# ttanida/rgrg

Measured on AMD Instinct MI355X. Metric: images/sec full 29-region report gen, 512x512 CXR, greedy max_len=128, higher is better.
Workload: dtype bf16; 1 GPU; full_model.generate() batch=32/GPU, 29 regions, greedy max_len=128, bf16 autocast: 16-bit detector, 16-bit decode GEMMs + K/V cache, hipGraph-captured decode step (BASELINE configs[2]); global_batch=32, parallelism=single GPU, weights=seeded random init (rgrg_amd.synth, profile bench), hipGraph_decode=True

## Files before the change

### include/rgrg_hip.h

```cpp
#ifndef RGRG_HIP_H_
#define RGRG_HIP_H_

#include <stdint.h>

#ifdef __cplusplus
extern "C" {
#endif

#define RGRG_OK 0
#define RGRG_EINVAL (-1)
#define RGRG_EHIP (-2)
#define RGRG_ESTATE (-3)

#define RGRG_ACT_NONE 0
#define RGRG_ACT_RELU 1
#define RGRG_ACT_GELU_NEW 2

const char* rgrg_last_error(void);
int rgrg_abi_version(void);
int rgrg_device_arch(int dev, char* buf, int buflen);

int rgrg_linear_f32(const float* A, const float* W, const float* scale, const float* shift, const float* R,
                    float* Y, int M, int N, int K, int ldy, int act, int splitk, float* ws, void* stream);
int rgrg_conv2d_nhwc_f32(const float* X, const float* W, const float* scale, const float* shift, const float* R,
// ... 143 lines not shown
int rgrg_linear_bf16w_f32(const float* A, const uint16_t* Wb, const float* shift, const float* R, float* Y, int M,
                          int N, int K, int ldy, int act, int fp16, void* stream);
int rgrg_linear_bf16_f32(const uint16_t* A16, const uint16_t* Wb, const float* shift, const float* R, float* Y,
                         uint16_t* Y16, int M, int N, int K, int ldy, int act, int fp16, void* stream);
int rgrg_debug_linear_bf16_tile(const uint16_t* A16, const uint16_t* Wb, const float* shift, const float* R, float* Y,
                                int M, int N, int K, int ldy, int act, int tile, int lda, int ldw, int fp16, void* stream);
int rgrg_debug_conv2d_nhwc_bf16_tile(const uint16_t* X16, const uint16_t* Wb, const float* shift, const uint16_t* R16, float* Y,
                                     uint16_t* Y16, int B, int H, int Wd, int Cin, int Cout, int KH, int KW, int stride,
                                     int pad, int act, int fp16, int tile, void* stream);
int rgrg_debug_bf16_tile_choice(int M, int N, int K);
int rgrg_debug_linear_bf16_train(const uint16_t* A16, const uint16_t* Wb, const float* shift, const float* R, float* Y,
                                 uint16_t* Y16, uint16_t* Ypre16, const uint16_t* G16, int M, int N, int K, int ldy, int act,
                                 int tile, int fp16, void* stream);
int rgrg_debug_linear_bf16_argmax(const uint16_t* A16, const uint16_t* Wb, const float* shift, int M, int N, int K,
                                  float* cand_val, int* cand_idx, int fp16, void* stream);
int rgrg_debug_ln_fold16(const float* w, const float* gain, const float* beta, const float* bias, uint16_t* wb, float* colsum,
                         float* shift, int N, int K, int fp16, void* stream);
int rgrg_debug_linear_bf16_ln(const uint16_t* A16, const uint16_t* Wb, const float* shift, const float* R, float* Y,
                              uint16_t* Yb16, float* stats_out, const float* ln_stats, const float* ln_colsum, int M, int N,
                              int K, int ldy, int act, int fp16, void* stream);
int rgrg_debug_linear_bf16_ln_kv(const uint16_t* A16, const uint16_t* Wb, const float* shift, float* Y, const float* ln_stats,
                                 const float* ln_colsum, uint16_t* kcache, uint16_t* vcache, const int* step_dev, int M, int H,
                                 int T_slots, int K, int ldy, int fp16, void* stream);
int rgrg_debug_linear_bf16_ln_kp(const uint16_t* A16, const uint16_t* Wb, const float* shift, const float* R, float* Y,
                                 uint16_t* Y16, uint16_t* Yb16, float* stats_out, const float* ln_stats, const float* ln_colsum,
                                 int M, int N, int K, int ldy, int act, int fp16, int kp, void* stream);
int rgrg_debug_wide_epilogue_launches(void);
int rgrg_debug_cons_epilogue_launches(void);
int rgrg_debug_attn_decode(const float* qkv, int ld_qkv, void* kcache, void* vcache, const int* step_dev, float* out,
                           uint16_t* out16, int S, int H, int T_slots, const int* src, const float* kmask, int kv16, int fp16,
// ... 98 lines not shown
```

### rgrg_amd/_hip.py

```python
from __future__ import annotations

import ctypes as C
import os
from typing import Optional

from . import build as _build

c_float_p = C.c_void_p
_i, _f, _p = C.c_int, C.c_float, C.c_void_p

ACT_NONE, ACT_RELU, ACT_GELU_NEW = 0, 1, 2
ABI_VERSION = 28


class RgrgHipError(RuntimeError):
    pass


class DecoderLayerWeights(C.Structure):
    _fields_ = [(n, _p) for n in ("ln1_g", "ln1_b", "ln2_g", "ln2_b", "c_attn_w", "c_attn_b", "attn_proj_w",
                                  "attn_proj_b", "c_fc_w", "c_fc_b", "mlp_proj_w", "mlp_proj_b")]


class DirectArgs(C.Structure):
# ... 63 lines not shown
    "rgrg_colsum_f32": (_i, [_p, _p, _i, _i, _p]),
    "rgrg_relu_backward_f32": (_i, [_p, _p, C.c_int64, _p]),
    "rgrg_bce_with_logits_masked_backward_f32": (_i, [_p, _p, _p, C.c_float, _i, C.c_float, _p, _i, _p]),
    "rgrg_adamw_step_f32": (_i, [_p, _p, _p, _p, C.c_int64, C.c_float, C.c_float, C.c_float, C.c_float, C.c_float, _i, C.c_float, _p]),
    "rgrg_adamw_multi_step_f32": (_i, [_p, _i, C.c_float, C.c_float, C.c_float, C.c_float, C.c_float, _i, C.c_float, _p]),
    "rgrg_f32_to_bf16": (_i, [_p, _p, C.c_int64, _i, _p]),
    "rgrg_bf16_to_f32": (_i, [_p, _p, C.c_int64, _i, _p]),
    "rgrg_conv2d_nhwc_bf16": (_i, [_p, _p, _p, _p, _p, _p, _i, _i, _i, _i, _i, _i, _i, _i, _i, _i, _i, _p]),
    "rgrg_linear_bf16w_f32": (_i, [_p, _p, _p, _p, _p, _i, _i, _i, _i, _i, _i, _p]),
    "rgrg_linear_bf16_f32": (_i, [_p, _p, _p, _p, _p, _p, _i, _i, _i, _i, _i, _i, _p]),
    "rgrg_debug_linear_bf16_tile": (_i, [_p, _p, _p, _p, _p, _i, _i, _i, _i, _i, _i, _i, _i, _i, _p]),
    "rgrg_debug_conv2d_nhwc_bf16_tile": (_i, [_p, _p, _p, _p, _p, _p, _i, _i, _i, _i, _i, _i, _i, _i, _i, _i, _i, _i, _p]),
    "rgrg_debug_bf16_tile_choice": (_i, [_i, _i, _i]),
    "rgrg_debug_linear_bf16_train": (_i, [_p, _p, _p, _p, _p, _p, _p, _p, _i, _i, _i, _i, _i, _i, _i, _p]),
    "rgrg_debug_linear_bf16_argmax": (_i, [_p, _p, _p, _i, _i, _i, _p, _p, _i, _p]),
    "rgrg_debug_ln_fold16": (_i, [_p, _p, _p, _p, _p, _p, _p, _i, _i, _i, _p]),
    "rgrg_debug_direct_pack": (_i, [_p, _p, _p, _p, _i, _i, _i, _p, _p, _p, _p, _p, _p]),
    "rgrg_debug_direct_linear": (_i, [C.POINTER(DirectArgs), _i, _i, _i, _i, C.POINTER(_i), _p]),
    "rgrg_debug_skinny_linear": (_i, [_p, _p, _p, _p, _p, _i, _i, _i, _i, _i, _p]),
    "rgrg_debug_linear_bf16_ln": (_i, [_p, _p, _p, _p, _p, _p, _p, _p, _p, _i, _i, _i, _i, _i, _i, _p]),
    "rgrg_debug_linear_bf16_ln_kp": (_i, [_p, _p, _p, _p, _p, _p, _p, _p, _p, _p, _i, _i, _i, _i, _i, _i, _i, _p]),
    "rgrg_debug_wide_epilogue_launches": (_i, []),
    "rgrg_debug_cons_epilogue_launches": (_i, []),
    "rgrg_debug_attn_decode": (_i, [_p, _i, _p, _p, _p, _p, _p, _i, _i, _i, _p, _p, _i, _i, _i, _i, _i, _p]),
    "rgrg_debug_linear_bf16_ln_kv": (_i, [_p, _p, _p, _p, _p, _p, _p, _p, _p, _i, _i, _i, _i, _i, _i, _p]),
    "rgrg_debug_attn_decode_qonly": (_i, [_p, _i, _p, _p, _p, _p, _p, _i, _i, _i, _i, _i, _p]),
    "rgrg_debug_attn_decode_first": (_i, [_p, _i, _p, _p, _p, _p, _p, _i, _i, _i, _p, _i, _i, _i, _p]),
    "rgrg_debug_attn_decode_rowstep": (_i, [_p, _i, _p, _p, _p, _p, _p, _i, _i, _i, _i, _i, _i, _i, _p]),
    "rgrg_debug_attn_decode_beam_first": (_i, [_p, _i, _p, _p, _p, _p, _p, _i, _i, _i, _p, _p, _i, _i, _i, _i, _p]),
    "rgrg_debug_attn_decode_kv8": (_i, [_p, _i, _p, _p, _p, _p, _p, _i, _i, _i, _p, _p, _i, _i, _p]),
# ... 82 lines not shown
```

### rgrg_amd/csrc/decoder.hip

```cpp
#include <math.h>
#include <stdlib.h>

#include <algorithm>
#include <type_traits>
#include <cmath>
#include <vector>

#include "decoder_internal.h"

namespace rgrg {

int skinny_max_rows() {
    static int v = -1;
    if (v < 0) { const char* e = getenv("RGRG_SKINNY_MAX_ROWS"); v = e ? atoi(e) : SKINNY_MAX_ROWS;
        if (v > SKINNY_MAX_ROWS) v = SKINNY_MAX_ROWS; if (v < 32) v = 32; }
    return v;
}

__global__ __launch_bounds__(256) void pack_weights_kernel(const float* __restrict__ W, float* __restrict__ P, int N,
                                                           int K, int NT) {
    const size_t total = (size_t)NT * (K / 8) * 64;
    for (size_t o = (size_t)blockIdx.x * blockDim.x + threadIdx.x; o < total; o += (size_t)gridDim.x * blockDim.x) {
        const int l = (int)(o & 63);
        const size_t t = o >> 6;
// ... 1184 lines not shown
    return kv_is_bf16(d, S) && d->xn16 && d->ln_fold && d->ln_stat && d->layers[0].c_attn.wb_ln && d->D == 1024;
}
static bool step_qkv_cache(const rgrg_decoder* d, const StepSpec& s) {
    const int S = s.rows;
    const KvFormat f = kv_format(d, S);
    const bool plain = !s.tok && !s.src;
    return d->qkv_cache && plain && step_ln_fold(d, S) && (f == KV_BF16 || f == KV_F16) && d->kp_gemms != 1 && d->kp_gemms != 3 && !s.key_mask;
}
static GemmLnFold cons_kv_cache(const rgrg_decoder* d, const GemmLnFold& cons, int l, int r0) {
    GemmLnFold f = cons;
    u16* kcr = reinterpret_cast<u16*>(d->kv) + (size_t)l * d->kv_layer_stride + (size_t)r0 * d->H * d->T * 64;
    f.kv_k = kcr; f.kv_v = kcr + d->kv_kv_stride; f.kv_step = d->step; f.kv_H = d->H; f.kv_T = d->T;
    return f;
}

static int enqueue_head(rgrg_decoder* d, int S, bool count, bool logits, unsigned short* xn16, bool roll = false) {
    hipStream_t st = d->stream;
    int rc;
    if (!logits && xn16 && lm_head_cand_path(d, S)) {
        GemmLnFold ce{};
        ce.cand_val = d->cand_val; ce.cand_idx = d->cand_idx;
        if ((rc = linear(d, d->lm_head, d->xn, nullptr, nullptr, S, d->ld_logits, RGRG_ACT_NONE, count, xn16, nullptr, &ce))) return rc;
        if ((rc = trace_mark(d, 0, 1002))) return rc;
        if (roll) return enqueue_roll_end(d, S, (d->lm_head.N + 255) / 256);
        hipLaunchKernelGGL(argmax_update_kernel, dim3(S), dim3(256), 0, st, d->cand_val, d->cand_idx, (d->lm_head.N + 255) / 256, d->ids,
                           d->max_len, d->finished, d->step, d->done_len, d->sync, S);
        RGRG_LAUNCH_CHECK();
        return trace_mark(d, 0, 1003);
    }
    if ((rc = linear(d, d->lm_head, d->xn, nullptr, d->logits, S, d->ld_logits, RGRG_ACT_NONE, count, xn16))) return rc;
    if (logits) return RGRG_OK;
    const int cand_nt = (d->V + 31) / 32;
    hipLaunchKernelGGL(logits_candidates_kernel, dim3(4, S), dim3(256), 0, st, d->logits, d->ld_logits, d->V,
                       cand_nt, d->cand_val, d->cand_idx);
    RGRG_LAUNCH_CHECK();
    if (roll) return enqueue_roll_end(d, S, cand_nt);
    hipLaunchKernelGGL(argmax_update_kernel, dim3(S), dim3(256), 0, st, d->cand_val, d->cand_idx, cand_nt, d->ids,
                       d->max_len, d->finished, d->step, d->done_len, d->sync, S);
    RGRG_LAUNCH_CHECK();
    return RGRG_OK;
// ... 66 lines not shown
            if (!fold) {
                if ((rc2 = launch_ln_rows(x, w.ln2_g, w.ln2_b, xn, D, xn16r, d->f16(), rows, rs))) return rc2;
            }
            if ((rc2 = linear(d, w.c_fc, xn, nullptr, d->ff + 4 * o, rows, 4 * D, RGRG_ACT_GELU_NEW, count, xn16r, ff16r, cfr))) return rc2;
            if ((rc2 = trace_mark(d, r0, l * 8 + 3))) return rc2;
            if ((rc2 = linear(d, w.mlp_proj, d->ff + 4 * o, x, x, rows, D, RGRG_ACT_NONE, count, ff16r, nullptr, pfr))) return rc2;
            if ((rc2 = trace_mark(d, r0, l * 8 + 4))) return rc2;
            if (!fold || l + 1 == d->n_layer) {
                if ((rc2 = launch_ln_rows(x, ng, nb, xn, D, xn16r, d->f16(), rows, rs))) return rc2;
                if ((rc2 = trace_mark(d, r0, 1001))) return rc2;
            }
        }
        return RGRG_OK;
    };
    if ((rc = run_row_ranges(d, S, step_chains(d, S, s.end == STEP_ARGMAX && !s.tok && !s.src, fold), run_rows))) return rc;
    return enqueue_head(d, S, count, s.end != STEP_ARGMAX && s.end != STEP_ROLL, xn16, s.end == STEP_ROLL);
}
int enqueue_step(rgrg_decoder* d, const StepSpec& s, bool count) {
    const int rc = s.rows <= decode_row_limit(d) ? enqueue_step_fused(d, s, count) : enqueue_step_tiled(d, s, count);
    if (rc) return rc;
    if (s.end == STEP_SAMPLE) return enqueue_sampler(d, s.rows);
    return s.end == STEP_ROLL_SAMPLE ? enqueue_roll_sample_end(d, s.rows) : RGRG_OK;
}

StepSpec padded_step_spec(rgrg_decoder* d, StepSpec s, const int* pad) {
    s.row_pos = d->row_pos;
    if (kv_format(d, s.rows) != KV_F32) s.kv_first = pad;
    else s.key_mask = d->key_mask;
    return s;
}

// ... 820 lines not shown
                }
                const GemmLnFold cons_kv = qc ? cons_kv_cache(d, cons_r, l, r0) : cons_r;
                if ((rc2 = linear(d, w.c_attn, d->xn + o, nullptr, d->qkv + 3 * o, rows, 3 * D, RGRG_ACT_NONE, c, xn16r, nullptr, qc ? &cons_kv : cfr))) break;
                if ((rc2 = linear(d, w.attn_proj, d->att + o, d->x + o, d->h1 + o, rows, D, RGRG_ACT_NONE, c, att16r, nullptr, pfr))) break;
                if ((rc2 = linear(d, w.c_fc, d->xn + o, nullptr, d->ff + 4 * o, rows, 4 * D, RGRG_ACT_GELU_NEW, c, xn16r, ff16r, cfr))) break;
                if ((rc2 = linear(d, w.mlp_proj, d->ff + 4 * o, d->x + o, d->h1 + o, rows, D, RGRG_ACT_NONE, c, ff16r, nullptr, pfr))) break;
            }
            return rc2;
        });
        if (!rc && fused) {
            DirectArgs h{};
            h.Xf = d->x; h.part = d->part; h.Y = d->logits; h.ldy = d->ld_logits; h.act = RGRG_ACT_NONE;
            rc = direct_linear(d, d->lm_head, h, DX_COMBINE4, S, c, true);
        } else if (!rc) {
            if (xn16 && lm_head_cand_path(d, S)) {
                GemmLnFold ce{};
                ce.cand_val = d->cand_val; ce.cand_idx = d->cand_idx;
                rc = linear(d, d->lm_head, d->xn, nullptr, nullptr, S, d->ld_logits, RGRG_ACT_NONE, c, xn16, nullptr, &ce);
            } else {
                rc = linear(d, d->lm_head, d->xn, nullptr, d->logits, S, d->ld_logits, RGRG_ACT_NONE, c, xn16);
            }
        }
    }
    if (!rc) {
        RGRG_HIP(hipEventRecord(e1, d->stream));
        RGRG_HIP(hipEventSynchronize(e1));
        RGRG_HIP(hipEventElapsedTime(&tg, e0, e1));
        hipLaunchKernelGGL(set_int_kernel, dim3(1), dim3(64), 0, d->stream, d->step, nkeys - 2);
        for (int it = -1; it < iters && !rc; ++it) {
            if (it == 0) RGRG_HIP(hipEventRecord(e0, d->stream));
            rc = run_row_ranges(d, S, fused ? 1 : step_chains(d, S, true, fold), [&](int r0, int rows) -> int {
                int rc2 = RGRG_OK;
                for (int l = 0; l < d->n_layer && !rc2; ++l)
// ... 53 lines not shown
```

### rgrg_amd/csrc/gemm_bf16.hip

```cpp
#include "gemm_bf16_device.h"

#include <atomic>

namespace rgrg {

struct GemmBf16Params {
    const float* A;
    const u16* A16;
    const u16* Wb;
    const float* shift;
    const float* R;
    float* Y;
    u16* Y16;
    int M, N, K, ldy, act;
    int lda = 0, ldw = 0;
    int cH = 0, cW = 0, cCin = 0, cKH = 0, cKW = 0, cStride = 1, cPad = 0, cOH = 0, cOW = 0;
    const u16* R16 = nullptr;
    int f16 = 0;
    u16* Yb16 = nullptr;
    float* stats_out = nullptr;
    const float* ln_stats = nullptr;
    const float* ln_colsum = nullptr;
    u16 *kv_k = nullptr, *kv_v = nullptr;
    const int* kv_step = nullptr;
    int kv_H = 0, kv_T = 0;
    u16* Ypre16 = nullptr;
    const u16* G16 = nullptr;
    int gm = 0;
    int ksplit = 0;
    float* sk_ws = nullptr;
    unsigned* sk_cnt = nullptr;
    float* cand_val = nullptr;
    int* cand_idx = nullptr;
    int dbg = 0;
};

constexpr int BK16 = 64;
constexpr int LDB = (BK16 * 2 + 16) / 2;

template <int BM, int BN, int THREADS, bool A16, bool F16>
__global__ __launch_bounds__(THREADS) void gemm_bf16w_kernel(const GemmBf16Params p, const int mtiles, const int ntiles) {
    constexpr int WAVES = THREADS / 64, WN = WAVES / 2;
    constexpr int TM = BM / 2, TN = BN / WN;
    constexpr int MI = TM / 32, NI = TN / 32;
    constexpr int AL = BM * 8 / THREADS, BL = BN * 8 / THREADS;
    constexpr int RSTEP = THREADS / 8;
    constexpr int NS = 4;
    extern __shared__ __attribute__((aligned(16))) u16 smem16[];
// ... 180 lines not shown
    __builtin_amdgcn_sched_group_barrier(0x008, MI * NI, 0);
    __builtin_amdgcn_sched_group_barrier(0x100, MI + NI, 0);
    __builtin_amdgcn_sched_group_barrier(0x008, MI * NI, 0);
    __builtin_amdgcn_sched_group_barrier(0x008, MI * NI, 0);
}

template <int BM, int BN, int NST, bool CONV, bool F16, int LNF, int CACT = -1>
__global__ __launch_bounds__(256) void gemm_bf16_glds_kernel(const GemmBf16Params p, const int mtiles, const int ntiles) {
    constexpr int BK = 64;
    constexpr int MI = BM / 64, NI = BN / 64;
    constexpr int LA = BM / 32, LB = BN / 32;
    constexpr int LPW = LA + LB;
    constexpr int STAGE = (BM + BN) * 128;
    static_assert((NST - 2) * LPW < 64, "counted vmcnt out of range");
    static_assert(NST >= 2 && NST <= 4, "tail is written for up to 3 trailing tiles");
    constexpr bool CONS = LNF >= 2, KVC = LNF == 3;
    static_assert(CACT == -1 || (CONS && BM == 64 && BN == 64), "compile-time activation: consumers on the 64 x 64 tile");
    constexpr int ETAG = (CACT + 1) * 256;
    extern __shared__ __attribute__((aligned(16))) unsigned char glds_smem[];
    const int tid = threadIdx.x, lane = tid & 63;
    const int wave = __builtin_amdgcn_readfirstlane(tid >> 6);
    const int wm = wave >> 1, wn = wave & 1;
    const int ks = (!CONV && p.ksplit > 1) ? p.ksplit : 1;
    const int t = xcd_band_tile(blockIdx.x, mtiles * ntiles * ks);
    const int slice = t % ks, tile = t / ks;
    const int2 tmn = grouped_tile(tile, p.gm, mtiles, ntiles);
    const int tm = tmn.x, tn = tmn.y;
    const int m0 = tm * BM, n0 = tn * BN;
    const int nk = p.K / BK / ks;
    const int lda = p.lda ? p.lda : p.K, ldw = p.ldw ? p.ldw : p.K;
    const u16* abase = CONV ? p.A16 - 128 : p.A16 + (size_t)m0 * lda + (size_t)slice * nk * BK;
    const u16* wbase = p.Wb + (size_t)n0 * ldw + (size_t)slice * nk * BK;
    const int lrow = lane >> 3, lch = lane & 7;
    int va[LA], vb[LB];
    int cy0[LA], cx0[LA], cpix[LA], cswz[LA];
#pragma unroll
    for (int j = 0; j < LA; ++j) {
        const int row = (j * 4 + wave) * 8 + lrow;
// ... 37 lines not shown
    for (int ks = 0; ks < 4; ++ks) foff[ks] = frag_offset(frow, fh, ks);

    f32x16 acc[MI][NI];
    zero_acc(acc);

    const int ccol = lane & 31, crow4 = 4 * (lane >> 5);
    float sh_pre[MI][NI], cs_pre[MI][NI];
#pragma unroll
    for (int mi = 0; mi < MI; ++mi)
#pragma unroll
        for (int ni = 0; ni < NI; ++ni) {
            const int colc = min(n0 + wn * (BN / 2) + ni * 32 + ccol, p.N - 1);
            sh_pre[mi][ni] = p.shift ? p.shift[colc] : 0.f;
            cs_pre[mi][ni] = CONS ? p.ln_colsum[colc] : 0.f;
        }
    constexpr bool PRE_R = MI * NI == 1 && !CONS;
    float rv_pre[16];
#pragma unroll
    for (int r = 0; r < 16; ++r) rv_pre[r] = 0.f;
    if constexpr (PRE_R) {
        if (p.R) {
            const int colc = min(n0 + wn * (BN / 2) + ccol, p.N - 1);
            const int rbase = m0 + wm * (BM / 2) + crow4;
#pragma unroll
            for (int r = 0; r < 16; ++r) rv_pre[r] = c_load_f32(p.R, rbase, r, colc, p.M, p.ldy);
        }
    }

    constexpr int TPR = 256 / BM, PER = 16 / TPR;
    f32x4 lsq[PER / 2];
    int kv_slot = 0;
// ... 23 lines not shown
        nxt = nxt + 1 == NST ? 0 : nxt + 1;
    }
#define RGRG_GLDS_TAIL(R)                                   \
    if constexpr (NST - 1 >= (R)) {                         \
        wait_vmcnt<((R) - 1) * LPW>();                      \
        __builtin_amdgcn_s_barrier();                       \
        __builtin_amdgcn_sched_barrier(0);                  \
        RGRG_GLDS_COMPUTE(cur);                             \
        cur = cur + 1 == NST ? 0 : cur + 1;                 \
    }
    RGRG_GLDS_TAIL(3) RGRG_GLDS_TAIL(2) RGRG_GLDS_TAIL(1)
#undef RGRG_GLDS_TAIL
#undef RGRG_GLDS_ISSUE
#undef RGRG_GLDS_COMPUTE

    if constexpr (!CONV) {
        if (ks > 1) {
            const __amdgpu_buffer_rsrc_t rs = bf16_rsrc(p.sk_ws + (size_t)tile * ks * (BM * BN));
            const int soff = slice * (BM * BN * 4);
#pragma unroll
            for (int mi = 0; mi < MI; ++mi)
#pragma unroll
                for (int ni = 0; ni < NI; ++ni)
#pragma unroll
                    for (int q = 0; q < 4; ++q)
                        __builtin_amdgcn_raw_buffer_store_b128(
                            __builtin_bit_cast(u32x4, f32x4{acc[mi][ni][4 * q], acc[mi][ni][4 * q + 1], acc[mi][ni][4 * q + 2], acc[mi][ni][4 * q + 3]}),
                            rs, (((mi * NI + ni) * 4 + q) * 256 + tid) * 16, soff, 16);
            asm volatile("s_waitcnt vmcnt(0)" ::: "memory");
            __syncthreads();
            unsigned* flag = reinterpret_cast<unsigned*>(glds_smem + NST * STAGE + BM * 8);
// ... 6 lines not shown
#pragma unroll
                for (int ni = 0; ni < NI; ++ni)
#pragma unroll
                    for (int q = 0; q < 4; ++q) {
                        f32x4 tot = {0.f, 0.f, 0.f, 0.f};
                        for (int sl = 0; sl < ks; ++sl) {
                            f32x4 v = __builtin_bit_cast(f32x4, __builtin_amdgcn_raw_buffer_load_b128(rs, (((mi * NI + ni) * 4 + q) * 256 + tid) * 16,
                                                                                                         sl * (BM * BN * 4), 16));
                            if (sl == slice) v = f32x4{acc[mi][ni][4 * q], acc[mi][ni][4 * q + 1], acc[mi][ni][4 * q + 2], acc[mi][ni][4 * q + 3]};
                            tot += v;
                        }
#pragma unroll
                        for (int e = 0; e < 4; ++e) acc[mi][ni][4 * q + e] = tot[e];
                    }
        }
    }

    float2* row_stat = reinterpret_cast<float2*>(glds_smem + NST * STAGE);
    if constexpr (CONS) {
        const float2 ls = ln_slot_sums<TPR, PER>(lsq);
        const float mean = ln_mean(ls.x), var = ln_var(ls.y, mean);
        if (tid % TPR == 0) row_stat[tid / TPR] = make_float2(mean, 1.0f / sqrtf(var + LN_EPS16));
        __syncthreads();
    }

    float blk1[MI], blk2[MI];
#pragma unroll
    for (int mi = 0; mi < MI; ++mi) { blk1[mi] = 0.f; blk2[mi] = 0.f; }
#pragma unroll
    for (int mi = 0; mi < MI; ++mi)
// ... 306 lines not shown
                cv[(g * 4 + wq) * 128 + lrow_t] = bv[0];
                ci[(g * 4 + wq) * 128 + lrow_t] = bi[0];
            }
        }
        __syncthreads();
        if (tid < 256) {
            const int gg = tid >> 7, lr = tid & 127, row = m0 + tid;
            float best = cv[(gg * 4) * 128 + lr];
            int idx = ci[(gg * 4) * 128 + lr];
#pragma unroll
            for (int q = 1; q < 4; ++q) {
                const float v = cv[(gg * 4 + q) * 128 + lr];
                if (v > best) { best = v; idx = ci[(gg * 4 + q) * 128 + lr]; }
            }
            if (row < p.M) {
                p.cand_val[(size_t)row * ntiles + tn] = best;
                p.cand_idx[(size_t)row * ntiles + tn] = idx;
            }
        }
        return;
    }
    const int ccol = lane & 31, crow4 = 4 * (lane >> 5);
#pragma unroll
    for (int mi = 0; mi < MI; ++mi)
#pragma unroll
        for (int ni = 0; ni < NI; ++ni) {
            const int col = n0 + wq * 64 + ni * 32 + ccol;
            const int colc = min(col, p.N - 1);
            const int rbase = m0 + g * 128 + mi * 32 + crow4;
            const float sh = esh[ni];
            float rv[16], vv[16];
#pragma unroll
// ... 83 lines not shown
    return e ? atoi(e) : 0;
}

typedef void (*gemm_kernel_t)(const GemmBf16Params, const int, const int);
struct GemmVariant {
    bool f16 = false;
    bool conv = false;
    int lnf = 0;
    int cact = -1;
    bool wide = false;
};
typedef gemm_kernel_t (*gemm_variant_fn)(const GemmVariant&);
static int set_dynamic_lds(gemm_variant_fn kernel_of, int lds) {
    for (int f16 = 0; f16 < 2; ++f16)
        for (int conv = 0; conv < 2; ++conv)
            for (int lnf = 0; lnf < 4; ++lnf)
                for (int cact : {-1, RGRG_ACT_NONE, RGRG_ACT_GELU_NEW})
                    for (int wide = 0; wide < 2; ++wide) {
                        const gemm_kernel_t k = kernel_of(GemmVariant{f16 != 0, conv != 0, lnf, cact, wide != 0});
                        if (k) RGRG_HIP(hipFuncSetAttribute(reinterpret_cast<const void*>(k), hipFuncAttributeMaxDynamicSharedMemorySize, lds));
                    }
    return RGRG_OK;
}
static int launch_variant(gemm_kernel_t k, int grid, int threads, int lds, const GemmBf16Params& p, int mtiles, int ntiles, hipStream_t st) {
    if (!k) { set_error("bf16 GEMM: this variant of the kernel is not instantiated"); return RGRG_EINVAL; }
    hipLaunchKernelGGL(k, dim3(grid), dim3(threads), lds, st, p, mtiles, ntiles);
    RGRG_LAUNCH_CHECK();
    return RGRG_OK;
}

template <int BM, int BN, int NST>
static gemm_kernel_t glds_kernel(const GemmVariant& v) {
#define RGRG_G_KERNEL(CONV_, ...) \
    (v.f16 ? gemm_bf16_glds_kernel<BM, BN, NST, CONV_, true, __VA_ARGS__> : gemm_bf16_glds_kernel<BM, BN, NST, CONV_, false, __VA_ARGS__>)
    if (v.wide) return nullptr;
    if (v.cact != -1) {
        if constexpr (BM == 64 && BN == 64) {
            if (!v.conv && v.lnf == 2 && v.cact == RGRG_ACT_NONE) return RGRG_G_KERNEL(false, 2, RGRG_ACT_NONE);
            if (!v.conv && v.lnf == 2 && v.cact == RGRG_ACT_GELU_NEW) return RGRG_G_KERNEL(false, 2, RGRG_ACT_GELU_NEW);
            if (!v.conv && v.lnf == 3 && v.cact == RGRG_ACT_NONE) return RGRG_G_KERNEL(false, 3, RGRG_ACT_NONE);
        }
        return nullptr;
    }
    if (v.conv) return v.lnf == 0 ? RGRG_G_KERNEL(true, 0) : nullptr;
    switch (v.lnf) {
        case 0: return RGRG_G_KERNEL(false, 0);
        case 1: return RGRG_G_KERNEL(false, 1);
        case 2: return RGRG_G_KERNEL(false, 2);
        case 3: return RGRG_G_KERNEL(false, 3);
    }
#undef RGRG_G_KERNEL
    return nullptr;
}
template <int BM, int BN, int NST>
constexpr int glds_lds() { return NST * (BM + BN) * 128 + BM * 16; }
template <int BM, int BN>
static int glds_attrs() {
    int rc;
    if ((rc = set_dynamic_lds(glds_kernel<BM, BN, 2>, glds_lds<BM, BN, 2>())) || (rc = set_dynamic_lds(glds_kernel<BM, BN, 3>, glds_lds<BM, BN, 3>()))) return rc;
    return set_dynamic_lds(glds_kernel<BM, BN, 4>, glds_lds<BM, BN, 4>());
}

#include "gemm_kp.inc"

constexpr int PP_LDS = 2 * (256 + 256) * 128;
static gemm_kernel_t pp_kernel(const GemmVariant& v) {
    if (v.conv || v.lnf != 0 || v.cact != -1 || v.wide) return nullptr;
    return v.f16 ? gemm_bf16_pp_kernel<true> : gemm_bf16_pp_kernel<false>;
}

int init_gemm_bf16_attrs() {
    static bool done = false;
    if (done) return RGRG_OK;
    int rc;
    if ((rc = bf16_attr<128, 128, 512>()) || (rc = bf16_attr<64, 64, 256>())) return rc;
    if ((rc = glds_attrs<128, 128>()) || (rc = glds_attrs<64, 64>()) || (rc = glds_attrs<128, 64>()) || (rc = glds_attrs<64, 128>())) return rc;
    if ((rc = set_dynamic_lds(pp_kernel, PP_LDS))) return rc;
    if ((rc = kp_attr<128, 128, 2>()) || (rc = kp_attr<64, 64, 4>()) || (rc = kp_attr<64, 64, 3>()) || (rc = kp_attr<128, 64, 3>()) || (rc = kp_attr<64, 128, 3>()) || (rc = kp_attr<64, 64, 2>()) || (rc = set_dynamic_lds(pr_kernel, PR_LDS))) return rc;
    done = true;
    return RGRG_OK;
}

static std::atomic<int> cons_epi_launches{0};
static bool cons_epi_enabled() {
    const char* e = getenv("RGRG_CONS_EPI");
    return !e || (atoi(e) & 1) != 0;
}
static bool cons_epi_ok(const GemmBf16Params& p) {
    const auto al = [](const void* q, uintptr_t a) { return (reinterpret_cast<uintptr_t>(q) & (a - 1)) == 0; };
// ... 8 lines not shown
    GemmBf16Params p = p0;
    const int mtiles = (p.M + BM - 1) / BM, ntiles = (p.N + BN - 1) / BN;
    if (p.gm == 0) p.gm = default_gm(mtiles, 16);
    const int ks = (!p.cCin && p.ksplit > 1 && p.sk_ws && p.sk_cnt && (p.K / 64) % p.ksplit == 0 && p.K / 64 / p.ksplit >= NST - 1) ? p.ksplit : 1;
    p.ksplit = ks;
    GemmVariant v;
    v.f16 = p.f16 != 0;
    bool cons = false;
    if constexpr (BM == 64 && BN == 64) cons = cons_epi_enabled() && cons_epi_ok(p);
    if (cons) {
        cons_epi_launches.fetch_add(1, std::memory_order_relaxed);
        v.lnf = p.kv_k ? 3 : 2;
        v.cact = p.act;
    }
    else if (p.cCin) v.conv = true;
    else if (p.Yb16) v.lnf = 1;
    else if (p.ln_colsum) v.lnf = p.kv_k ? 3 : 2;
    return launch_variant(glds_kernel<BM, BN, NST>(v), mtiles * ntiles * ks, 256, glds_lds<BM, BN, NST>(), p, mtiles, ntiles, st);
}
template <int BM, int BN>
static int launch_glds_nst(const GemmBf16Params& p, int nst, hipStream_t st) {
    if (nst == 2) return launch_glds_cfg<BM, BN, 2>(p, st);
    if (nst == 3) return launch_glds_cfg<BM, BN, 3>(p, st);
    return launch_glds_cfg<BM, BN, 4>(p, st);
}

static bool pp_eligible(const GemmBf16Params& p) {
    return !p.cCin && !p.Yb16 && !p.ln_colsum && !p.R16 && p.K >= 256 && p.K % 64 == 0;
}
static int launch_pp(const GemmBf16Params& p0, hipStream_t st) {
// ... 63 lines not shown
    nst = glds_stages(nst, p.K);
    switch (shape) {
        case 1: return launch_glds_nst<128, 128>(p, nst, st);
        case 2: return launch_glds_nst<64, 64>(p, nst, st);
        case 3: return launch_glds_nst<128, 64>(p, nst, st);
        case 4: return launch_glds_nst<64, 128>(p, nst, st);
    }
    set_error("bf16 GEMM: unknown tile configuration %d", tile);
    return RGRG_EINVAL;
}

bool gemm_bf16_cand_epilogue_ok(int M, int N, int K) {
    static const bool on = [] { const char* e = getenv("RGRG_LMHEAD_CAND"); return !e || atoi(e) != 0; }();
    const long tiles_pp = (long)((M + 255) / 256) * ((N + 255) / 256);
    return on && pp_enabled() && pp_lm_head() && M >= 512 && N >= 32768 && tiles_pp >= 512 && K >= 256 && K % 64 == 0;
}

int launch_gemm_bf16w_ex(const float* A, const void* A16, const void* Wb, const float* shift, const float* R, float* Y, void* Y16,
                         int M, int N, int K, int ldy, int act, hipStream_t st, int f16, const GemmLnFold* ln) {
    RGRG_CHECK_ARG((A || A16) && Wb && (Y || Y16 || (ln && ln->cand_val)) && M > 0 && N > 0 && K > 0 && K % (4 * BK16) == 0 && ldy >= N);
    GemmBf16Params p{A, reinterpret_cast<const u16*>(A16), reinterpret_cast<const u16*>(Wb), shift, R, Y,
                     reinterpret_cast<u16*>(Y16), M, N, K, ldy, act};
    p.f16 = f16 ? 1 : 0;
    if (ln && (ln->Ypre16 || ln->G16)) {
        RGRG_CHECK_ARG(A16 && (size_t)128 * K * 2 < ((size_t)1 << 31) && !ln->Yb16 && !ln->ln_colsum);
        RGRG_CHECK_ARG(!(ln->Ypre16 && ln->G16) && (!ln->G16 || (!R && act == RGRG_ACT_NONE)));
        p.Ypre16 = reinterpret_cast<u16*>(ln->Ypre16); p.G16 = reinterpret_cast<const u16*>(ln->G16);
    } else if (ln && (ln->Yb16 || ln->ln_colsum)) {
        RGRG_CHECK_ARG(A16 && (size_t)128 * K * 2 < ((size_t)1 << 31));
        RGRG_CHECK_ARG((ln->Yb16 != nullptr) != (ln->ln_colsum != nullptr));
// ... 2 lines not shown
        p.Yb16 = reinterpret_cast<u16*>(ln->Yb16); p.stats_out = ln->stats_out;
        p.ln_stats = ln->ln_stats; p.ln_colsum = ln->ln_colsum;
        if (ln->kv_k) {
            RGRG_CHECK_ARG(ln->ln_colsum && ln->kv_v && ln->kv_step && ln->kv_H > 0 && ln->kv_T >= 2 && N == 3 * ln->kv_H * 64 && Y && !Y16 && !ln->kp &&
                           ln->ksplit <= 1 && act == RGRG_ACT_NONE);
            p.kv_k = reinterpret_cast<u16*>(ln->kv_k); p.kv_v = reinterpret_cast<u16*>(ln->kv_v);
            p.kv_step = ln->kv_step; p.kv_H = ln->kv_H; p.kv_T = ln->kv_T;
        }
    } else if (ln && ln->kv_k) {
        set_error("bf16 GEMM: the K/V-cache epilogue belongs to the folded-LayerNorm consumer");
        return RGRG_EINVAL;
    }
    if (ln && ln->ksplit > 1) { p.ksplit = ln->ksplit; p.sk_ws = ln->sk_ws; p.sk_cnt = ln->sk_cnt; }
    if (ln && ln->cand_val) {
        RGRG_CHECK_ARG(A16 && ln->cand_idx && !R && act == RGRG_ACT_NONE && !Y16 && !ln->Yb16 && !ln->ln_colsum && !ln->Ypre16 && !ln->G16);
        p.cand_val = ln->cand_val; p.cand_idx = ln->cand_idx;
        return launch_glds(p, 5, st);
    }
    if (ln && ln->kp && A16 && (size_t)128 * K * 2 < ((size_t)1 << 31) && kp_eligible(p, 4)) return launch_glds(p, 11, st);
    if (A16 && (size_t)128 * K * 2 < ((size_t)1 << 31)) return launch_glds(p, 0, st);
    const long tiles_big = (long)((M + 127) / 128) * ((N + 127) / 128);
    return tiles_big >= 192 ? launch_bf16_cfg<128, 128, 512>(p, st) : launch_bf16_cfg<64, 64, 256>(p, st);
}

int launch_gemm_bf16w(const float* A, const void* Wb, const float* shift, const float* R, float* Y, int M, int N, int K,
                      int ldy, int act, hipStream_t st, int f16) {
    return launch_gemm_bf16w_ex(A, nullptr, Wb, shift, R, Y, nullptr, M, N, K, ldy, act, st, f16, nullptr);
}

__global__ __launch_bounds__(256) void bf16_to_f32_kernel(const u16* __restrict__ src, float* __restrict__ dst, size_t n, int f16) {
    for (size_t i = (size_t)blockIdx.x * blockDim.x + threadIdx.x; i < n; i += (size_t)gridDim.x * blockDim.x)
// ... 59 lines not shown
    RGRG_CHECK_ARG((size_t)128 * K * 2 < ((size_t)1 << 31) && !(Ypre16 && G16) && (!G16 || (!R && act == RGRG_ACT_NONE)));
    GemmBf16Params p{nullptr, A16, Wb, shift, R, Y, Y16, M, N, K, ldy, act};
    p.f16 = fp16 ? 1 : 0;
    p.Ypre16 = Ypre16; p.G16 = G16;
    return launch_glds(p, tile, as_stream(stream));
}

extern "C" int rgrg_debug_linear_bf16_argmax(const uint16_t* A16, const uint16_t* Wb, const float* shift, int M, int N, int K,
                                             float* cand_val, int* cand_idx, int fp16, void* stream) {
    int rc = init_gemm_bf16_attrs();
    if (rc) return rc;
    RGRG_CHECK_ARG(A16 && Wb && cand_val && cand_idx && M > 0 && N > 0 && K >= 256 && K % 256 == 0);
    GemmLnFold f{};
    f.cand_val = cand_val; f.cand_idx = cand_idx;
    return launch_gemm_bf16w_ex(nullptr, A16, Wb, shift, nullptr, nullptr, nullptr, M, N, K, N, RGRG_ACT_NONE, as_stream(stream), fp16, &f);
}

extern "C" int rgrg_debug_linear_bf16_ln(const uint16_t* A16, const uint16_t* Wb, const float* shift, const float* R, float* Y,
                                         uint16_t* Yb16, float* stats_out, const float* ln_stats, const float* ln_colsum, int M,
                                         int N, int K, int ldy, int act, int fp16, void* stream) {
    int rc = init_gemm_bf16_attrs();
    if (rc) return rc;
    RGRG_CHECK_ARG(A16 && Wb && Y);
    GemmLnFold f{};
    f.Yb16 = Yb16; f.stats_out = stats_out; f.ln_stats = ln_stats; f.ln_colsum = ln_colsum;
    return launch_gemm_bf16w_ex(nullptr, A16, Wb, shift, R, Y, nullptr, M, N, K, ldy, act, as_stream(stream), fp16, &f);
}

extern "C" int rgrg_debug_linear_bf16_ln_kv(const uint16_t* A16, const uint16_t* Wb, const float* shift, float* Y, const float* ln_stats,
                                            const float* ln_colsum, uint16_t* kcache, uint16_t* vcache, const int* step_dev, int M, int H,
// ... 63 lines not shown
```

### rgrg_amd/csrc/gemm_bf16_device.h

```cpp
#pragma once
#include "internal.h"

namespace rgrg {

typedef short bf16x8 __attribute__((ext_vector_type(8)));
typedef short bf16x4 __attribute__((ext_vector_type(4)));
typedef unsigned short u16;
typedef __attribute__((address_space(3))) void* lds_ptr_t;

constexpr float LN_EPS16 = 1e-5f;

template <bool F16>
__device__ __forceinline__ f32x16 mfma16(const bf16x8& a, const bf16x8& b, const f32x16& c) {
    if constexpr (F16) return __builtin_amdgcn_mfma_f32_32x32x16_f16(__builtin_bit_cast(f16x8, a), __builtin_bit_cast(f16x8, b), c, 0, 0, 0);
    else return __builtin_amdgcn_mfma_f32_32x32x16_bf16(a, b, c, 0, 0, 0);
}

__device__ __forceinline__ __amdgpu_buffer_rsrc_t bf16_rsrc(const void* p) {
    return __builtin_amdgcn_make_buffer_rsrc(const_cast<void*>(p), 0, 0x7fffffff, 0x00020000);
}

template <int N>
__device__ __forceinline__ void wait_vmcnt() {
    static_assert(N >= 0 && N < 64, "vmcnt is a 6-bit field");
// ... 65 lines not shown
}
template <bool F16>
__device__ __forceinline__ float c_load_16(const u16* src, int rbase, int r, int colc, int M, int ld) {
    const int row = min(c_row(r, rbase), M - 1);
    return from16<F16>(src[(size_t)row * ld + colc]);
}
__device__ __forceinline__ size_t c_offset(int rbase, int r, int col, int ld) { return (size_t)rbase * ld + col + (size_t)(c_row(r) * ld); }
template <bool F16, bool STREAM, bool YB>
__device__ __forceinline__ void c_store(size_t o, float v, u16* Y16, int N, float* Y, u16* Yb16) {
    if (Y16) Y16[o] = (u16)to16<F16>(v);
    else if (STREAM && N > 8192) __builtin_nontemporal_store(v, &Y[o]);
    else Y[o] = v;
    if constexpr (YB) Yb16[o] = (u16)to16<F16>(v);
}

template <int TPR, int PER>
__device__ __forceinline__ float2 ln_slot_sums(const f32x4 (&lsq)[PER / 2]) {
    static_assert(TPR * PER == 16 && (PER == 4 || PER == 8), "slot reduction is written for 64- and 128-row tiles");
    float ls1 = 0.f, ls2 = 0.f;
#pragma unroll
    for (int j0 = 0; j0 < PER / 2; j0 += 2) {
        float g1 = 0.f, g2 = 0.f;
#pragma unroll
        for (int j = j0; j < j0 + 2; ++j) { g1 += lsq[j][0]; g2 += lsq[j][1]; g1 += lsq[j][2]; g2 += lsq[j][3]; }
        if (j0 == 0) { ls1 = g1; ls2 = g2; } else { ls1 += g1; ls2 += g2; }
    }
#pragma unroll
    for (int o = 1; o < TPR; o <<= 1) { ls1 += __shfl_xor(ls1, o, 64); ls2 += __shfl_xor(ls2, o, 64); }
    return make_float2(ls1, ls2);
}
// ... 8 lines not shown
    {                                                                                     \
        const bool up = (lane & (BIT)) != 0;                                              \
        _Pragma("unroll") for (int i = 0; i < (H); ++i) {                                 \
            const float s1 = up ? a1[i] : a1[i + (H)], s2 = up ? a2[i] : a2[i + (H)];     \
            const float k1 = up ? a1[i + (H)] : a1[i], k2 = up ? a2[i + (H)] : a2[i];     \
            a1[i] = k1 + __shfl_xor(s1, (BIT), 64);                                       \
            a2[i] = k2 + __shfl_xor(s2, (BIT), 64);                                       \
        }                                                                                 \
    }
    RGRG_BFLY(8, 16) RGRG_BFLY(4, 8) RGRG_BFLY(2, 4) RGRG_BFLY(1, 2)
#undef RGRG_BFLY
    a1[0] += __shfl_xor(a1[0], 1, 64);
    a2[0] += __shfl_xor(a2[0], 1, 64);
    return make_float2(a1[0], a2[0]);
}
__device__ __forceinline__ int ln_block_sum_row(int lane) { return c_row((lane >> 1) & 15) + 4 * (lane >> 5); }
template <int MI>
__device__ __forceinline__ void ln_stats_hand_over(float2* xch, int w, int lrow, const float (&blk1)[MI], const float (&blk2)[MI]) {
#pragma unroll
    for (int mi = 0; mi < MI; ++mi) xch[(w * MI + mi) * 32 + lrow] = make_float2(blk1[mi], blk2[mi]);
}
template <int MI, int NI>
__device__ __forceinline__ void ln_stats_store(const float2* xch, int w, int lrow, const float (&blk1)[MI], const float (&blk2)[MI], int row0,
                                               int slot, int M, float* stats_out) {
#pragma unroll
    for (int mi = 0; mi < MI; ++mi) {
        float s1 = blk1[mi], s2 = blk2[mi];
        if constexpr (NI == 1) {
            const float2 o = xch[((w + 1) * MI + mi) * 32 + lrow];
            s1 += o.x; s2 += o.y;
        }
// ... 7 lines not shown
```

### rgrg_amd/csrc/internal.h

```cpp
#pragma once
#include "common.h"

namespace rgrg {

int launch_gemm_dense(const float* A, const float* W, const float* shift, const float* R, float* Y, int M, int N, int K,
                      int ldy, int act, float* ws, size_t ws_floats, hipStream_t st);
int init_gemm_attrs();

struct GemmLnFold {
    void* Yb16 = nullptr;
    float* stats_out = nullptr;
    const float* ln_stats = nullptr;
    const float* ln_colsum = nullptr;
    void* Ypre16 = nullptr;
    const void* G16 = nullptr;
    int ksplit = 0;
    float* sk_ws = nullptr;
    unsigned* sk_cnt = nullptr;
    float* cand_val = nullptr;
    int* cand_idx = nullptr;
    int kp = 0;
    void *kv_k = nullptr, *kv_v = nullptr;
    const int* kv_step = nullptr;
    int kv_H = 0, kv_T = 0;
};
int init_gemm_bf16_attrs();
bool gemm_bf16_cand_epilogue_ok(int M, int N, int K);
int launch_gemm_bf16w_ex(const float* A, const void* A16, const void* Wb, const float* shift, const float* R, float* Y, void* Y16,
                         int M, int N, int K, int ldy, int act, hipStream_t st, int f16, const GemmLnFold* ln = nullptr);
int launch_gemm_bf16w(const float* A, const void* Wb, const float* shift, const float* R, float* Y, int M, int N, int K,
                      int ldy, int act, hipStream_t st, int f16);
int convert_f32_to_bf16(const float* src, void* dst, size_t n, hipStream_t st, int f16);

int launch_gelu_apply(const float* pre, float* out, size_t n, hipStream_t st);
int launch_gelu_backward(float* d, const float* pre, size_t n, hipStream_t st);
int launch_relu_backward(float* d, const float* h, size_t n, hipStream_t st);
int launch_ln_backward(const float* dy, const float* x, const float* g, float* out, int rows, int D, int accumulate, hipStream_t st);
int launch_ce_backward(float* logits, size_t ld, int V, int row0, int rows, const long long* ids, const int* row_valid,
                       const float* row_lse, const int* n_scored, float scale, const int* id_error, hipStream_t st);
int launch_transpose_pad(const float* src, float* dst, int R, int Cc, int Rp, hipStream_t st);
int launch_colsum(const float* src, float* out, int R, int Cc, hipStream_t st);
int launch_attn_backward(const float* qkv, const float* ukv, int ld_ukv, int kcol, const float* am, const float* d_att,
// ... 26 lines not shown
```

Baseline: 90.74 images/sec.

## Split LM-head argmax GEMM into full-wave main part and small-tile tail

The fused LM-head GEMM with argmax-candidate epilogue is split along N. The main part runs on the 256x256 kernel over a column count chosen so its tile count divides into whole rounds across the device's CUs. The leftover vocabulary columns go to a second launch on 64x64 tiles with a new candidate epilogue that does a butterfly row max. This targets the partially filled last wave of the large-tile launch during greedy decode. In exchange it adds a kernel launch per step and more candidate slots for the argmax reduction to scan.

```diff
diff --git a/include/rgrg_hip.h b/include/rgrg_hip.h
--- a/include/rgrg_hip.h
+++ b/include/rgrg_hip.h
@@ -181,6 +181,9 @@
                                  int tile, int fp16, void* stream);
 int rgrg_debug_linear_bf16_argmax(const uint16_t* A16, const uint16_t* Wb, const float* shift, int M, int N, int K,
                                   float* cand_val, int* cand_idx, int fp16, void* stream);
+int rgrg_debug_linear_bf16_argmax_split(const uint16_t* A16, const uint16_t* Wb, const float* shift, int M, int N, int K, int split,
+                                        float* cand_val, int* cand_idx, int ld_cand, int fp16, void* stream);
+int rgrg_debug_lm_head_split(int M, int N);
 int rgrg_debug_ln_fold16(const float* w, const float* gain, const float* beta, const float* bias, uint16_t* wb, float* colsum,
                          float* shift, int N, int K, int fp16, void* stream);
 int rgrg_debug_linear_bf16_ln(const uint16_t* A16, const uint16_t* Wb, const float* shift, const float* R, float* Y,
diff --git a/rgrg_amd/_hip.py b/rgrg_amd/_hip.py
--- a/rgrg_amd/_hip.py
+++ b/rgrg_amd/_hip.py
@@ -101,6 +101,8 @@
     "rgrg_debug_bf16_tile_choice": (_i, [_i, _i, _i]),
     "rgrg_debug_linear_bf16_train": (_i, [_p, _p, _p, _p, _p, _p, _p, _p, _i, _i, _i, _i, _i, _i, _i, _p]),
     "rgrg_debug_linear_bf16_argmax": (_i, [_p, _p, _p, _i, _i, _i, _p, _p, _i, _p]),
+    "rgrg_debug_linear_bf16_argmax_split": (_i, [_p, _p, _p, _i, _i, _i, _i, _p, _p, _i, _i, _p]),
+    "rgrg_debug_lm_head_split": (_i, [_i, _i]),
     "rgrg_debug_ln_fold16": (_i, [_p, _p, _p, _p, _p, _p, _p, _i, _i, _i, _p]),
     "rgrg_debug_direct_pack": (_i, [_p, _p, _p, _p, _i, _i, _i, _p, _p, _p, _p, _p, _p]),
     "rgrg_debug_direct_linear": (_i, [C.POINTER(DirectArgs), _i, _i, _i, _i, C.POINTER(_i), _p]),
diff --git a/rgrg_amd/csrc/decoder.hip b/rgrg_amd/csrc/decoder.hip
--- a/rgrg_amd/csrc/decoder.hip
+++ b/rgrg_amd/csrc/decoder.hip
@@ -1222,16 +1222,25 @@
     return f;
 }
 
-static int enqueue_head(rgrg_decoder* d, int S, bool count, bool logits, unsigned short* xn16, bool roll = false) {
+static int lm_head_cand_launch(rgrg_decoder* d, int S, bool count, unsigned short* xn16, bool rounds, int* cand_nt) {
+    GemmLnFold ce{};
+    ce.cand_val = d->cand_val; ce.cand_idx = d->cand_idx;
+    ce.cand_split = rounds ? gemm_bf16_cand_split(S, d->lm_head.N) : 0;
+    *cand_nt = gemm_bf16_cand_count(d->lm_head.N, ce.cand_split);
+    if (*cand_nt > d->lm_head.NT) ce.cand_split = 0, *cand_nt = gemm_bf16_cand_count(d->lm_head.N, 0);
+    if (count && ce.cand_split) d->gemm_launches_per_step += 1;
+    return linear(d, d->lm_head, d->xn, nullptr, nullptr, S, d->ld_logits, RGRG_ACT_NONE, count, xn16, nullptr, &ce);
+}
+
+static int enqueue_head(rgrg_decoder* d, int S, bool count, bool logits, unsigned short* xn16, bool roll = false, bool rounds = false) {
     hipStream_t st = d->stream;
     int rc;
     if (!logits && xn16 && lm_head_cand_path(d, S)) {
-        GemmLnFold ce{};
-        ce.cand_val = d->cand_val; ce.cand_idx = d->cand_idx;
-        if ((rc = linear(d, d->lm_head, d->xn, nullptr, nullptr, S, d->ld_logits, RGRG_ACT_NONE, count, xn16, nullptr, &ce))) return rc;
+        int cand_nt = 0;
+        if ((rc = lm_head_cand_launch(d, S, count, xn16, rounds && !roll, &cand_nt))) return rc;
         if ((rc = trace_mark(d, 0, 1002))) return rc;
-        if (roll) return enqueue_roll_end(d, S, (d->lm_head.N + 255) / 256);
-        hipLaunchKernelGGL(argmax_update_kernel, dim3(S), dim3(256), 0, st, d->cand_val, d->cand_idx, (d->lm_head.N + 255) / 256, d->ids,
+        if (roll) return enqueue_roll_end(d, S, cand_nt);
+        hipLaunchKernelGGL(argmax_update_kernel, dim3(S), dim3(256), 0, st, d->cand_val, d->cand_idx, cand_nt, d->ids,
                            d->max_len, d->finished, d->step, d->done_len, d->sync, S);
         RGRG_LAUNCH_CHECK();
         return trace_mark(d, 0, 1003);
@@ -1328,7 +1337,8 @@
         return RGRG_OK;
     };
     if ((rc = run_row_ranges(d, S, step_chains(d, S, s.end == STEP_ARGMAX && !s.tok && !s.src, fold), run_rows))) return rc;
-    return enqueue_head(d, S, count, s.end != STEP_ARGMAX && s.end != STEP_ROLL, xn16, s.end == STEP_ROLL);
+    const bool plain_greedy = s.end == STEP_ARGMAX && !s.tok && !s.src && !s.row_pos;
+    return enqueue_head(d, S, count, s.end != STEP_ARGMAX && s.end != STEP_ROLL, xn16, s.end == STEP_ROLL, plain_greedy && fold);
 }
 int enqueue_step(rgrg_decoder* d, const StepSpec& s, bool count) {
     const int rc = s.rows <= decode_row_limit(d) ? enqueue_step_fused(d, s, count) : enqueue_step_tiled(d, s, count);
@@ -2179,9 +2189,8 @@
             rc = direct_linear(d, d->lm_head, h, DX_COMBINE4, S, c, true);
         } else if (!rc) {
             if (xn16 && lm_head_cand_path(d, S)) {
-                GemmLnFold ce{};
-                ce.cand_val = d->cand_val; ce.cand_idx = d->cand_idx;
-                rc = linear(d, d->lm_head, d->xn, nullptr, nullptr, S, d->ld_logits, RGRG_ACT_NONE, c, xn16, nullptr, &ce);
+                int cand_nt = 0;
+                rc = lm_head_cand_launch(d, S, c, xn16, fold, &cand_nt);
             } else {
                 rc = linear(d, d->lm_head, d->xn, nullptr, d->logits, S, d->ld_logits, RGRG_ACT_NONE, c, xn16);
             }
diff --git a/rgrg_amd/csrc/gemm_bf16.hip b/rgrg_amd/csrc/gemm_bf16.hip
--- a/rgrg_amd/csrc/gemm_bf16.hip
+++ b/rgrg_amd/csrc/gemm_bf16.hip
@@ -32,6 +32,7 @@
     unsigned* sk_cnt = nullptr;
     float* cand_val = nullptr;
     int* cand_idx = nullptr;
+    int cand_ld = 0, cand_col0 = 0;
     int dbg = 0;
 };
 
@@ -242,14 +243,15 @@
     constexpr int STAGE = (BM + BN) * 128;
     static_assert((NST - 2) * LPW < 64, "counted vmcnt out of range");
     static_assert(NST >= 2 && NST <= 4, "tail is written for up to 3 trailing tiles");
-    constexpr bool CONS = LNF >= 2, KVC = LNF == 3;
+    constexpr bool CONS = LNF == 2 || LNF == 3, KVC = LNF == 3, CAND = LNF == 4;
     static_assert(CACT == -1 || (CONS && BM == 64 && BN == 64), "compile-time activation: consumers on the 64 x 64 tile");
+    static_assert(!CAND || (BM == 64 && BN == 64 && !CONV), "candidate epilogue: 64 x 64 tile");
     constexpr int ETAG = (CACT + 1) * 256;
     extern __shared__ __attribute__((aligned(16))) unsigned char glds_smem[];
     const int tid = threadIdx.x, lane = tid & 63;
     const int wave = __builtin_amdgcn_readfirstlane(tid >> 6);
     const int wm = wave >> 1, wn = wave & 1;
-    const int ks = (!CONV && p.ksplit > 1) ? p.ksplit : 1;
+    const int ks = (!CONV && !CAND && p.ksplit > 1) ? p.ksplit : 1;
     const int t = xcd_band_tile(blockIdx.x, mtiles * ntiles * ks);
     const int slice = t % ks, tile = t / ks;
     const int2 tmn = grouped_tile(tile, p.gm, mtiles, ntiles);
@@ -317,7 +319,7 @@
             sh_pre[mi][ni] = p.shift ? p.shift[colc] : 0.f;
             cs_pre[mi][ni] = CONS ? p.ln_colsum[colc] : 0.f;
         }
-    constexpr bool PRE_R = MI * NI == 1 && !CONS;
+    constexpr bool PRE_R = MI * NI == 1 && !CONS && !CAND;
     float rv_pre[16];
 #pragma unroll
     for (int r = 0; r < 16; ++r) rv_pre[r] = 0.f;
@@ -371,7 +373,7 @@
 #undef RGRG_GLDS_ISSUE
 #undef RGRG_GLDS_COMPUTE
 
-    if constexpr (!CONV) {
+    if constexpr (!CONV && !CAND) {
         if (ks > 1) {
             const __amdgpu_buffer_rsrc_t rs = bf16_rsrc(p.sk_ws + (size_t)tile * ks * (BM * BN));
             const int soff = slice * (BM * BN * 4);
@@ -408,6 +410,35 @@
                         for (int e = 0; e < 4; ++e) acc[mi][ni][4 * q + e] = tot[e];
                     }
         }
+    }
+
+    if constexpr (CAND) {
+        const int c0 = n0 + wn * 32 + ccol;
+        float bv[16];
+        int bi[16];
+#pragma unroll
+        for (int r = 0; r < 16; ++r) {
+            bv[r] = c0 < p.N ? acc[0][0][r] + sh_pre[0][0] : -INFINITY;
+            bi[r] = p.cand_col0 + c0;
+        }
+        cand_block_row_max(bv, bi, lane);
+        float* cv = reinterpret_cast<float*>(glds_smem + NST * STAGE);
+        int* ci = reinterpret_cast<int*>(glds_smem + NST * STAGE + 2 * BM * 4);
+        if (!(lane & 1)) {
+            const int lrow = wm * 32 + ln_block_sum_row(lane);
+            cv[wn * BM + lrow] = bv[0];
+            ci[wn * BM + lrow] = bi[0];
+        }
+        __syncthreads();
+        if (tid < BM && m0 + tid < p.M) {
+            float best = cv[tid];
+            int idx = ci[tid];
+            if (cv[BM + tid] > best) { best = cv[BM + tid]; idx = ci[BM + tid]; }
+            const int cld = p.cand_ld ? p.cand_ld : ntiles;
+            p.cand_val[(size_t)(m0 + tid) * cld + tn] = best;
+            p.cand_idx[(size_t)(m0 + tid) * cld + tn] = idx;
+        }
+        return;
     }
 
     float2* row_stat = reinterpret_cast<float2*>(glds_smem + NST * STAGE);
@@ -744,8 +775,9 @@
                 if (v > best) { best = v; idx = ci[(gg * 4 + q) * 128 + lr]; }
             }
             if (row < p.M) {
-                p.cand_val[(size_t)row * ntiles + tn] = best;
-                p.cand_idx[(size_t)row * ntiles + tn] = idx;
+                const int cld = p.cand_ld ? p.cand_ld : ntiles;
+                p.cand_val[(size_t)row * cld + tn] = best;
+                p.cand_idx[(size_t)row * cld + tn] = idx;
             }
         }
         return;
@@ -859,7 +891,7 @@
 static int set_dynamic_lds(gemm_variant_fn kernel_of, int lds) {
     for (int f16 = 0; f16 < 2; ++f16)
         for (int conv = 0; conv < 2; ++conv)
-            for (int lnf = 0; lnf < 4; ++lnf)
+            for (int lnf = 0; lnf < 5; ++lnf)
                 for (int cact : {-1, RGRG_ACT_NONE, RGRG_ACT_GELU_NEW})
                     for (int wide = 0; wide < 2; ++wide) {
                         const gemm_kernel_t k = kernel_of(GemmVariant{f16 != 0, conv != 0, lnf, cact, wide != 0});
@@ -888,6 +920,10 @@
         return nullptr;
     }
     if (v.conv) return v.lnf == 0 ? RGRG_G_KERNEL(true, 0) : nullptr;
+    if (v.lnf == 4) {
+        if constexpr (BM == 64 && BN == 64 && NST == 4) return RGRG_G_KERNEL(false, 4);
+        return nullptr;
+    }
     switch (v.lnf) {
         case 0: return RGRG_G_KERNEL(false, 0);
         case 1: return RGRG_G_KERNEL(false, 1);
@@ -914,10 +950,12 @@
     return v.f16 ? gemm_bf16_pp_kernel<true> : gemm_bf16_pp_kernel<false>;
 }
 
+static int device_cus();
 int init_gemm_bf16_attrs() {
     static bool done = false;
     if (done) return RGRG_OK;
     int rc;
+    (void)device_cus();
     if ((rc = bf16_attr<128, 128, 512>()) || (rc = bf16_attr<64, 64, 256>())) return rc;
     if ((rc = glds_attrs<128, 128>()) || (rc = glds_attrs<64, 64>()) || (rc = glds_attrs<128, 64>()) || (rc = glds_attrs<64, 128>())) return rc;
     if ((rc = set_dynamic_lds(pp_kernel, PP_LDS))) return rc;
@@ -956,6 +994,7 @@
         v.cact = p.act;
     }
     else if (p.cCin) v.conv = true;
+    else if (p.cand_val) v.lnf = 4;
     else if (p.Yb16) v.lnf = 1;
     else if (p.ln_colsum) v.lnf = p.kv_k ? 3 : 2;
     return launch_variant(glds_kernel<BM, BN, NST>(v), mtiles * ntiles * ks, 256, glds_lds<BM, BN, NST>(), p, mtiles, ntiles, st);
@@ -1049,6 +1088,46 @@
     static const bool on = [] { const char* e = getenv("RGRG_LMHEAD_CAND"); return !e || atoi(e) != 0; }();
     const long tiles_pp = (long)((M + 255) / 256) * ((N + 255) / 256);
     return on && pp_enabled() && pp_lm_head() && M >= 512 && N >= 32768 && tiles_pp >= 512 && K >= 256 && K % 64 == 0;
+}
+
+static int device_cus() {
+    static const int n = [] {
+        int dev = 0, v = 0;
+        if (hipGetDevice(&dev) != hipSuccess || hipDeviceGetAttribute(&v, hipDeviceAttributeMultiprocessorCount, dev) != hipSuccess) v = 0;
+        return v;
+    }();
+    return n;
+}
+int gemm_bf16_cand_split(int M, int N) {
+    const char* e = getenv("RGRG_LMHEAD_ROUNDS");
+    const int sw = e ? atoi(e) : 1;
+    const int cus = sw > 1 ? sw : (sw == 1 ? device_cus() : 0);
+    if (cus <= 0) return 0;
+    const int mtiles = (M + 255) / 256;
+    int g = cus;
+    for (int a = mtiles % cus; a; ) { const int t = g % a; g = a; a = t; }
+    const int step = cus / g, n_main = N / 256 / step * step;
+    return (n_main > 0 && n_main * 256 < N) ? n_main * 256 : 0;
+}
+int gemm_bf16_cand_count(int N, int split) { return split > 0 ? split / 256 + (N - split + 63) / 64 : (N + 255) / 256; }
+
+static int launch_cand_split(const GemmBf16Params& p0, int split, hipStream_t st) {
+    GemmBf16Params p = p0;
+    RGRG_CHECK_ARG(split > 0 && split % 256 == 0 && split < p.N && !p.lda && !p.ldw);
+    const int n_main = split / 256, n_all = gemm_bf16_cand_count(p.N, split);
+    if (!p.cand_ld) p.cand_ld = n_all;
+    RGRG_CHECK_ARG(p.cand_ld >= n_all);
+    GemmBf16Params m = p;
+    m.N = split;
+    if (!pp_eligible(m)) { set_error("bf16 GEMM: the 256 x 256 kernel does not take this variant"); return RGRG_EINVAL; }
+    const int rc = launch_pp(m, st);
+    if (rc) return rc;
+    GemmBf16Params r = p;
+    r.Wb = p.Wb + (size_t)split * p.K;
+    r.shift = p.shift ? p.shift + split : nullptr;
+    r.N = p.N - split;
+    r.cand_val = p.cand_val + n_main; r.cand_idx = p.cand_idx + n_main; r.cand_col0 = split;
+    return launch_glds_cfg<64, 64, 4>(r, st);
 }
 
 int launch_gemm_bf16w_ex(const float* A, const void* A16, const void* Wb, const float* shift, const float* R, float* Y, void* Y16,
@@ -1081,7 +1160,8 @@
     if (ln && ln->ksplit > 1) { p.ksplit = ln->ksplit; p.sk_ws = ln->sk_ws; p.sk_cnt = ln->sk_cnt; }
     if (ln && ln->cand_val) {
         RGRG_CHECK_ARG(A16 && ln->cand_idx && !R && act == RGRG_ACT_NONE && !Y16 && !ln->Yb16 && !ln->ln_colsum && !ln->Ypre16 && !ln->G16);
-        p.cand_val = ln->cand_val; p.cand_idx = ln->cand_idx;
+        p.cand_val = ln->cand_val; p.cand_idx = ln->cand_idx; p.cand_ld = ln->cand_ld;
+        if (ln->cand_split) return launch_cand_split(p, ln->cand_split, st);
         return launch_glds(p, 5, st);
     }
     if (ln && ln->kp && A16 && (size_t)128 * K * 2 < ((size_t)1 << 31) && kp_eligible(p, 4)) return launch_glds(p, 11, st);
@@ -1171,6 +1251,21 @@
     GemmLnFold f{};
     f.cand_val = cand_val; f.cand_idx = cand_idx;
     return launch_gemm_bf16w_ex(nullptr, A16, Wb, shift, nullptr, nullptr, nullptr, M, N, K, N, RGRG_ACT_NONE, as_stream(stream), fp16, &f);
+}
+
+extern "C" int rgrg_debug_linear_bf16_argmax_split(const uint16_t* A16, const uint16_t* Wb, const float* shift, int M, int N, int K,
+                                                   int split, float* cand_val, int* cand_idx, int ld_cand, int fp16, void* stream) {
+    int rc = init_gemm_bf16_attrs();
+    if (rc) return rc;
+    RGRG_CHECK_ARG(A16 && Wb && cand_val && cand_idx && M > 0 && N > 0 && K >= 256 && K % 256 == 0 && (size_t)128 * K * 2 < ((size_t)1 << 31));
+    RGRG_CHECK_ARG(split >= 0 && split % 256 == 0 && split < N && ld_cand >= gemm_bf16_cand_count(N, split));
+    GemmLnFold f{};
+    f.cand_val = cand_val; f.cand_idx = cand_idx; f.cand_split = split; f.cand_ld = ld_cand;
+    return launch_gemm_bf16w_ex(nullptr, A16, Wb, shift, nullptr, nullptr, nullptr, M, N, K, N, RGRG_ACT_NONE, as_stream(stream), fp16, &f);
+}
+extern "C" int rgrg_debug_lm_head_split(int M, int N) {
+    RGRG_CHECK_ARG(M > 0 && N > 0);
+    return gemm_bf16_cand_split(M, N);
 }
 
 extern "C" int rgrg_debug_linear_bf16_ln(const uint16_t* A16, const uint16_t* Wb, const float* shift, const float* R, float* Y,
diff --git a/rgrg_amd/csrc/gemm_bf16_device.h b/rgrg_amd/csrc/gemm_bf16_device.h
--- a/rgrg_amd/csrc/gemm_bf16_device.h
+++ b/rgrg_amd/csrc/gemm_bf16_device.h
@@ -103,6 +103,29 @@
     if constexpr (YB) Yb16[o] = (u16)to16<F16>(v);
 }
 
+__device__ __forceinline__ int ln_block_sum_row(int lane) { return c_row((lane >> 1) & 15) + 4 * (lane >> 5); }
+
+__device__ __forceinline__ void cand_block_row_max(float (&bv)[16], int (&bi)[16], int lane) {
+#define RGRG_CAND_BFLY(H, BIT)                                                                \
+    {                                                                                         \
+        const bool up = (lane & (BIT)) != 0;                                                  \
+        _Pragma("unroll") for (int j = 0; j < (H); ++j) {                                     \
+            const float keep_v = up ? bv[j + (H)] : bv[j], send_v = up ? bv[j] : bv[j + (H)]; \
+            const int keep_i = up ? bi[j + (H)] : bi[j], send_i = up ? bi[j] : bi[j + (H)];   \
+            const float ov = __shfl_xor(send_v, (BIT), 64);                                   \
+            const int oi = __shfl_xor(send_i, (BIT), 64);                                     \
+            const bool take = ov > keep_v || (ov == keep_v && oi < keep_i);                   \
+            bv[j] = take ? ov : keep_v;                                                       \
+            bi[j] = take ? oi : keep_i;                                                       \
+        }                                                                                     \
+    }
+    RGRG_CAND_BFLY(8, 16) RGRG_CAND_BFLY(4, 8) RGRG_CAND_BFLY(2, 4) RGRG_CAND_BFLY(1, 2)
+#undef RGRG_CAND_BFLY
+    const float ov = __shfl_xor(bv[0], 1, 64);
+    const int oi = __shfl_xor(bi[0], 1, 64);
+    if (ov > bv[0] || (ov == bv[0] && oi < bi[0])) { bv[0] = ov; bi[0] = oi; }
+}
+
 template <int TPR, int PER>
 __device__ __forceinline__ float2 ln_slot_sums(const f32x4 (&lsq)[PER / 2]) {
     static_assert(TPR * PER == 16 && (PER == 4 || PER == 8), "slot reduction is written for 64- and 128-row tiles");
@@ -141,7 +164,6 @@
     a2[0] += __shfl_xor(a2[0], 1, 64);
     return make_float2(a1[0], a2[0]);
 }
-__device__ __forceinline__ int ln_block_sum_row(int lane) { return c_row((lane >> 1) & 15) + 4 * (lane >> 5); }
 template <int MI>
 __device__ __forceinline__ void ln_stats_hand_over(float2* xch, int w, int lrow, const float (&blk1)[MI], const float (&blk2)[MI]) {
 #pragma unroll
diff --git a/rgrg_amd/csrc/internal.h b/rgrg_amd/csrc/internal.h
--- a/rgrg_amd/csrc/internal.h
+++ b/rgrg_amd/csrc/internal.h
@@ -19,6 +19,8 @@
     unsigned* sk_cnt = nullptr;
     float* cand_val = nullptr;
     int* cand_idx = nullptr;
+    int cand_split = 0;
+    int cand_ld = 0;
     int kp = 0;
     void *kv_k = nullptr, *kv_v = nullptr;
     const int* kv_step = nullptr;
@@ -26,6 +28,8 @@
 };
 int init_gemm_bf16_attrs();
 bool gemm_bf16_cand_epilogue_ok(int M, int N, int K);
+int gemm_bf16_cand_split(int M, int N);
+int gemm_bf16_cand_count(int N, int split);
 int launch_gemm_bf16w_ex(const float* A, const void* A16, const void* Wb, const float* shift, const float* R, float* Y, void* Y16,
                          int M, int N, int K, int ldy, int act, hipStream_t st, int f16, const GemmLnFold* ln = nullptr);
 int launch_gemm_bf16w(const float* A, const void* Wb, const float* shift, const float* R, float* Y, int M, int N, int K,
```

Result: no change. 91.00 images/sec, median of 6 (+0.3%).
